# MarioAriasC/corda

Hardware: AMD Instinct MI355X
Metric: Ed25519 verifies/sec (node) (higher is better)
Workload: dtype uint32/uint64 (GF(2^255-19) radix 2^25.5 limbs, v_mad_u64_u32); 1 GPU; C2: 1M single-signer Ed25519 txs, 300-byte msg, distinct keys, SoA batch; sigs_per_gpu=1000000, msg_bytes=300, key_pool=distinct, parallelism=shard-by-signature x1, device_streams=2, gpu_max_hw_queues=4, collective=none

## Files before the change

### corda_amd/csrc/cv_field.h

```cpp
#pragma once
#include <hip/hip_runtime.h>
#include <stdint.h>
#include "cv_madc.h"

#define CV_HD __host__ __device__ __forceinline__

#if defined(CV_BOUNDS_CHECK) && !defined(__HIP_DEVICE_COMPILE__)
#include <cstdio>
#include <cstdlib>
#define CV_ASSERT(c, msg)                                                  \
    do {                                                                   \
        if (!(c)) {                                                        \
            fprintf(stderr, "cv_field bound violated: %s (%s:%d)\n", msg, __FILE__, __LINE__); \
            abort();                                                       \
        }                                                                  \
    } while (0)
#define CV_CHECKING 1
#else
#define CV_ASSERT(c, msg) ((void)0)
#define CV_CHECKING 0
#endif

struct fe { uint32_t v[10]; };

#define CV_W(i) (((i) & 1) ? 25 : 26)
#define CV_MASK(i) (((i) & 1) ? 0x1ffffffu : 0x3ffffffu)

#define CV_KP0(k) ((uint32_t)(k) * 0x3ffffedu)
#define CV_KPO(k) ((uint32_t)(k) * 0x1ffffffu)
#define CV_KPE(k) ((uint32_t)(k) * 0x3ffffffu)
CV_HD uint32_t cv_kp(int k, int i) { return i == 0 ? CV_KP0(k) : ((i & 1) ? CV_KPO(k) : CV_KPE(k)); }

CV_HD void fe_zero(fe &h) {
#pragma unroll
    for (int i = 0; i < 10; i++) h.v[i] = 0;
}
CV_HD void fe_one(fe &h) { fe_zero(h); h.v[0] = 1; }
CV_HD void fe_add(fe &h, const fe &f, const fe &g) {
#pragma unroll
    for (int i = 0; i < 10; i++) h.v[i] = f.v[i] + g.v[i];
}
template <int K> CV_HD void fe_sub(fe &h, const fe &f, const fe &g) {
#pragma unroll
    for (int i = 0; i < 10; i++) {
        CV_ASSERT(g.v[i] <= cv_kp(K, i), "fe_sub: subtrahend limb exceeds k*p");
        uint32_t k = cv_kp(K, i);
        const uint32_t x = g.v[i];
#ifdef __HIP_DEVICE_COMPILE__
        asm("" : "+s"(k));
#endif
        h.v[i] = (k > x ? k - x : x - k) + f.v[i];
    }
}
template <int K> CV_HD void fe_sub_carry_even(fe &h, const fe &f, const fe &g) {
#pragma unroll
    for (int i = 0; i < 10; i += 2) {
        uint32_t k0 = cv_kp(K, i), k1 = cv_kp(K, i + 1);
        CV_ASSERT(g.v[i] <= k0 && g.v[i + 1] <= k1, "fe_sub: subtrahend limb exceeds k*p");
#ifdef __HIP_DEVICE_COMPILE__
        asm("" : "+s"(k0), "+s"(k1));
#endif
        const uint32_t x0 = g.v[i], x1 = g.v[i + 1];
        const uint32_t e = (k0 > x0 ? k0 - x0 : x0 - k0) + f.v[i];
        uint32_t a1 = f.v[i + 1] + (e >> 26);
#ifdef __HIP_DEVICE_COMPILE__
        asm("" : "+v"(a1));
#endif
        h.v[i] = e & 0x3ffffffu;
        h.v[i + 1] = (k1 > x1 ? k1 - x1 : x1 - k1) + a1;
    }
}

CV_HD void fe_neg(fe &h, const fe &f) {
#pragma unroll
// ... 434 lines not shown
```

### corda_amd/csrc/cv_group.h

```cpp
#pragma once
#include "cv_field.h"

struct ge_p2 { fe X, Y, Z; };
struct ge_p3 { fe X, Y, Z, T; };
struct ge_p1p1 { fe X, Y, Z, T; };
struct ge_cached { fe YplusX, YminusX, Z, T2d; };
struct ge_precomp { fe yplusx, yminusx, xy2d; };

#define CV_FE_D   {56195235, 13857412, 51736253, 6949390, 114729, 24766616, 60832955, 30306712, 48412415, 21499315}
#define CV_FE_D2  {45281625, 27714825, 36363642, 13898781, 229458, 15978800, 54557047, 27058993, 29715967, 9444199}
#define CV_FE_SQRTM1 {34513072, 25610706, 9377949, 3500415, 12389472, 33281959, 41962654, 31548777, 326685, 11406482}

CV_HD void fe_const_d(fe &h) { const fe c = {CV_FE_D}; h = c; }
CV_HD void fe_const_d2(fe &h) { const fe c = {CV_FE_D2}; h = c; }
CV_HD void fe_const_sqrtm1(fe &h) { const fe c = {CV_FE_SQRTM1}; h = c; }

CV_HD void ge_p3_identity(ge_p3 &r) { fe_zero(r.X); fe_one(r.Y); fe_one(r.Z); fe_zero(r.T); }
CV_HD void ge_p2_identity(ge_p2 &r) { fe_zero(r.X); fe_one(r.Y); fe_one(r.Z); }
CV_HD void ge_cached_identity(ge_cached &r) { fe_one(r.YplusX); fe_one(r.YminusX); fe_one(r.Z); fe_zero(r.T2d); }
CV_HD void ge_precomp_identity(ge_precomp &r) { fe_one(r.yplusx); fe_one(r.yminusx); fe_zero(r.xy2d); }

CV_HD void ge_p1p1_to_p2(ge_p2 &r, const ge_p1p1 &p) {
    fe h[3];
    const fe f[3] = {p.T, p.Y, p.T}, g[3] = {p.X, p.Z, p.Z};
    fe_mul_n<3>(h, f, g);
    r.X = h[0]; r.Y = h[1]; r.Z = h[2];
}
CV_HD void ge_p1p1_to_p3(ge_p3 &r, const ge_p1p1 &p) {
    fe h[4];
    const fe f[4] = {p.T, p.Y, p.T, p.Y}, g[4] = {p.X, p.Z, p.Z, p.X};
    fe_mul_n<4>(h, f, g);
    r.X = h[0]; r.Y = h[1]; r.Z = h[2]; r.T = h[3];
}
CV_HD void ge_p3_to_p2(ge_p2 &r, const ge_p3 &p) { r.X = p.X; r.Y = p.Y; r.Z = p.Z; }
CV_HD void ge_p3_to_cached(ge_cached &r, const ge_p3 &p) {
    fe d2;
    fe_const_d2(d2);
    fe_add(r.YplusX, p.Y, p.X);
    fe_sub<2>(r.YminusX, p.Y, p.X);
    r.Z = p.Z;
    fe_mul(r.T2d, p.T, d2);
}

CV_HD void ge_p2_dbl(ge_p1p1 &r, const ge_p2 &p) {
    fe a, sq[4];
    fe_add(a, p.X, p.Y);
    const fe in[4] = {p.X, p.Y, p.Z, a};
    fe_sq_n<4, 0x4>(sq, in);
    const fe &xx = sq[0], &yy = sq[1], &zz2 = sq[2], &aa = sq[3];
    fe_add(r.Y, yy, xx);
    fe_sub<2>(r.Z, yy, xx);
    fe_sub_carry_even<3>(r.X, aa, r.Y);
    fe_sub<4>(r.T, zz2, r.Z);
}
CV_HD void ge_p3_dbl(ge_p1p1 &r, const ge_p3 &p) {
    ge_p2 q;
    ge_p3_to_p2(q, p);
    ge_p2_dbl(r, q);
}

CV_HD void ge_add(ge_p1p1 &r, const ge_p3 &p, const ge_cached &q) {
    fe s, d, m[4];
    fe_add(s, p.Y, p.X);
    fe_sub<2>(d, p.Y, p.X);
    const fe f[4] = {q.YplusX, q.YminusX, q.T2d, p.Z}, g[4] = {s, d, p.T, q.Z};
    fe_mul_n<4>(m, f, g);
    const fe &a = m[0], &b = m[1], &c = m[2];
    fe dd;
    fe_add(dd, m[3], m[3]);
    fe_sub<2>(r.X, a, b);
    fe_add(r.Y, a, b);
    fe_add(r.Z, dd, c);
    fe_sub<2>(r.T, dd, c);
}
CV_HD void ge_madd(ge_p1p1 &r, const ge_p3 &p, const ge_precomp &q) {
    fe s, d, m[3], dd;
    fe_add(s, p.Y, p.X);
    fe_sub<2>(d, p.Y, p.X);
    const fe f[3] = {q.yplusx, q.yminusx, q.xy2d}, g[3] = {s, d, p.T};
    fe_mul_n<3>(m, f, g);
    const fe &a = m[0], &b = m[1], &c = m[2];
    fe_add(dd, p.Z, p.Z);
    fe_sub<2>(r.X, a, b);
    fe_add(r.Y, a, b);
    fe_add(r.Z, dd, c);
    fe_sub<2>(r.T, dd, c);
}

CV_HD void ge_cached_cneg(ge_cached &r, bool neg) {
    fe a = r.YplusX, b = r.YminusX;
    fe_sel(r.YplusX, a, b, neg);
    fe_sel(r.YminusX, b, a, neg);
    uint32_t m = neg ? 0xffffffffu : 0u;
#ifdef __HIP_DEVICE_COMPILE__
    asm("" : "+v"(m));
#endif
#pragma unroll
    for (int i = 0; i < 10; i++) {
        CV_ASSERT(r.T2d.v[i] <= cv_kp(2, i), "ge_cached_cneg: 2dT limb exceeds 2p");
        r.T2d.v[i] = (r.T2d.v[i] ^ m) + (m & (cv_kp(2, i) + 1u));
    }
}
CV_HD void ge_precomp_cneg(ge_precomp &r, bool neg) {
    fe a = r.yplusx, b = r.yminusx, t;
    fe_sel(r.yplusx, a, b, neg);
    fe_sel(r.yminusx, b, a, neg);
    fe_neg(t, r.xy2d);
    fe_sel(r.xy2d, r.xy2d, t, neg);
}

__host__ __device__ __forceinline__ void ge_p2_encode(uint32_t w[8], const ge_p2 &p) {
    fe zi, x, y;
    fe_invert(zi, p.Z);
    fe_mul(x, p.X, zi);
    fe_mul(y, p.Y, zi);
    uint32_t xw[8];
    fe_to_words(w, y);
    fe_to_words(xw, x);
    w[7] |= (xw[0] & 1u) << 31;
}

CV_HD void ge_abyte_from_key(uint32_t abyte[8], const uint32_t w[8]) {
// ... 160 lines not shown
```

### corda_amd/csrc/cv_k_hs.hip

```cpp
#include "cv_kcommon.h"

template <int WAVES>
__global__ __launch_bounds__(CV_BLOCK, WAVES) void cv_scalars_kernel(uint32_t n, uint32_t cap, const uint8_t *__restrict__ pk,
                                                                 const uint8_t *__restrict__ sig,
                                                                 const uint8_t *__restrict__ arena,
                                                                 const uint64_t *__restrict__ off,
                                                                 const uint32_t *__restrict__ len,
                                                                 uint32_t *__restrict__ ws_dig) {
    const uint32_t i = blockIdx.x * CV_BLOCK + threadIdx.x;
    if (i < n) cv_scalars_lane<false, true>(i, cap, pk, sig, arena, off, len, ws_dig);
}

template <int WAVES, bool SUB>
__global__ __launch_bounds__(CV_BLOCK, WAVES) void cv_points_one_kernel(uint32_t n, const uint8_t *__restrict__ pk,
                                                                        const uint8_t *__restrict__ sig,
                                                                        uint32_t *__restrict__ ws_tab,
                                                                        uint32_t *__restrict__ ws_tabR,
                                                                        uint8_t *__restrict__ ws_ok,
                                                                        uint8_t *__restrict__ status) {
    cv_points_one_lane(blockIdx.x * CV_BLOCK + threadIdx.x, n, pk, sig, ws_tab, ws_tabR, ws_ok, status);
}

__global__ __launch_bounds__(CV_BLOCK) void cv_bw16_init_kernel(uint32_t *__restrict__ tab) {
    __shared__ __attribute__((aligned(16))) uint32_t btab[CV_BTAB_ENTRIES * CV_BTAB_STRIDE];
    stage_btab(btab);
    const uint32_t t = blockIdx.x * CV_BLOCK + threadIdx.x;
    if (t >= CV_BW16_ROWS * CV_BW16_ENTRIES) return;
    const uint32_t row = t / CV_BW16_ENTRIES, k = t % CV_BW16_ENTRIES;
    uint32_t sc[8] = {0, 0, 0, 0, 0, 0, 0, 0};
#pragma unroll
    for (int q = 0; q < 4; q++) sc[2 * q] = (uint32_t)q == row ? k : 0u;
    ge_p3 P;
    ge_scalarmult_base(P, sc, btab);
    fe zi, x, y, xy, d2, f[3];
    fe_invert(zi, P.Z);
    fe_mul(x, P.X, zi);
    fe_mul(y, P.Y, zi);
    fe_add(f[0], y, x);
    fe_sub<2>(f[1], y, x);
    fe_mul(xy, x, y);
    fe_const_d2(d2);
    fe_mul(f[2], xy, d2);
    uint32_t *o = tab + (size_t)t * CV_BTAB_STRIDE;
#pragma unroll
    for (int c = 0; c < 3; c++) {
        uint32_t w[8];
        fe_to_words(w, f[c]);
        fe canon;
        fe_from_words(canon, w);
        fe_store(o + 10 * c, canon);
    }
    o[30] = o[31] = 0;
}
template __global__ void cv_points_one_kernel<3, false>(uint32_t n, const uint8_t *pk, const uint8_t *sig, uint32_t *ws_tab, uint32_t *ws_tabR, uint8_t *ws_ok, uint8_t *status);
template __global__ void cv_points_one_kernel<3, true>(uint32_t n, const uint8_t *pk, const uint8_t *sig, uint32_t *ws_tab, uint32_t *ws_tabR, uint8_t *ws_ok, uint8_t *status);
template __global__ void cv_scalars_kernel<3>(uint32_t n, uint32_t cap, const uint8_t *pk, const uint8_t *sig, const uint8_t *arena, const uint64_t *off, const uint32_t *len, uint32_t *ws_dig);
```

### corda_amd/csrc/cv_kcommon.h

```cpp
#pragma once
#include <hip/hip_runtime.h>
#include <stdint.h>

#include "cv_verify.h"
#include "cv_quad.h"
#include "cv_hsquad.h"

#define CV_BLOCK 256
#ifndef CV_HSS_WAVES
#define CV_HSS_WAVES 3
#endif

__device__ __forceinline__ void stage_btab(uint32_t *lds) {
    for (int i = threadIdx.x; i < CV_BTAB_ENTRIES * CV_BTAB_STRIDE; i += blockDim.x) lds[i] = CV_BTAB[i];
    __syncthreads();
}

__device__ __forceinline__ void load_words8(uint32_t w[8], const uint8_t *p) {
    const uint4 a = reinterpret_cast<const uint4 *>(p)[0];
    const uint4 b = reinterpret_cast<const uint4 *>(p)[1];
    w[0] = a.x; w[1] = a.y; w[2] = a.z; w[3] = a.w;
    w[4] = b.x; w[5] = b.y; w[6] = b.z; w[7] = b.w;
}


__device__ __forceinline__ void store_words(uint32_t *dst, const uint32_t *src, int nwords4) {
    uint4 *d = reinterpret_cast<uint4 *>(dst);
#pragma unroll
    for (int q = 0; q < nwords4; q++) d[q] = make_uint4(src[4 * q], src[4 * q + 1], src[4 * q + 2], src[4 * q + 3]);
}

template <bool B16 = false, bool W16 = false>
__device__ __forceinline__ void cv_scalars_lane(uint32_t i, uint32_t cap, const uint8_t *pk, const uint8_t *sig,
                                                const uint8_t *arena, const uint64_t *off, const uint32_t *len,
                                                uint32_t *ws_dig) {
    uint32_t aw[8], rw[8], sw[8];
    load_words8(aw, pk + (size_t)i * 32);
    load_words8(rw, sig + (size_t)i * 64);
    load_words8(sw, sig + (size_t)i * 64 + 32);
    uint32_t hs[CV_HS_WORDS];
    cv_keyed_hs(aw, rw, sw, arena + off[i], len[i], hs);
    cv_hs_scalars<B16, W16>(hs, ws_dig + i, cap);
}

template <bool LAT = true>
__device__ __forceinline__ void cv_points_pair_lane(uint32_t g, uint32_t n, const uint8_t *pk, const uint8_t *sig,
                                                    uint32_t *ws_tab, uint32_t *ws_tabR, uint8_t *ws_ok,
                                                    uint8_t *status) {
    const uint32_t i = g >> 1;
    if (i >= n) return;
    const bool is_r = (g & 1u) != 0;
    uint32_t w[8];
    load_words8(w, is_r ? sig + (size_t)i * 64 : pk + (size_t)i * 32);
    const bool ok = cv_hs_point_one<LAT>(w, is_r, (is_r ? ws_tabR : ws_tab) + (size_t)i * CV_TAB_WORDS);
    const bool r_ok = __shfl_xor((int)ok, 1) != 0;
    if (!is_r) {
        ws_ok[i] = (ok && r_ok) ? 1 : 0;
        if (status) status[i] = ok ? 0 : 1;
    }
}

template <bool LAT = true>
__device__ __forceinline__ void cv_points_quad_lane(uint32_t g, uint32_t n, const uint8_t *pk, const uint8_t *sig,
                                                    uint32_t *ws_tab, uint32_t *ws_tabR, uint8_t *ws_ok,
                                                    uint8_t *status) {
    const uint32_t i = g >> 2;
    if (i >= n) return;
    const bool is_r = (g & 1u) != 0;
    const int half = (int)((g >> 1) & 1u);
    uint32_t w[8];
    load_words8(w, is_r ? sig + (size_t)i * 64 : pk + (size_t)i * 32);
    const bool ok = cv_hs_point_one<LAT>(w, is_r, (is_r ? ws_tabR : ws_tab) + (size_t)i * CV_TAB_WORDS, half);
    const bool r_ok = __shfl_xor((int)ok, 1) != 0;
    if (!is_r && half == 0) {
        ws_ok[i] = (ok && r_ok) ? 1 : 0;
        if (status) status[i] = ok ? 0 : 1;
    }
}

__device__ __forceinline__ void cv_points_one_lane(uint32_t g, uint32_t n, const uint8_t *pk, const uint8_t *sig,
                                                   uint32_t *ws_tab, uint32_t *ws_tabR, uint8_t *ws_ok,
                                                   uint8_t *status) {
    const uint32_t i = g >> 1;
    if (i >= n) return;
    const bool is_r = (g & 1u) != 0;
    uint32_t w[8];
    load_words8(w, is_r ? sig + (size_t)i * 64 : pk + (size_t)i * 32);
    const bool ok = cv_hs_point_one<false>(w, is_r, (is_r ? ws_tabR : ws_tab) + (size_t)i * CV_TAB_WORDS);
    const bool r_ok = __shfl_xor((int)ok, 1) != 0;
    if (!is_r) {
        ws_ok[i] = (ok && r_ok) ? 1 : 0;
        if (status) status[i] = ok ? 0 : 1;
    }
}
// ... 25 lines not shown
```

### corda_amd/csrc/cv_kernels.hip

```cpp
#include <hip/hip_runtime.h>
#include <stdint.h>

#include <mutex>

#include "cv_kcommon.h"
#include "cv_launch.h"

static uint32_t *g_bw16[64];
static std::mutex g_bw16_mu;
static hipError_t bw16_table(const uint32_t **out, hipStream_t st) {
    int dev = 0;
    hipError_t e = hipGetDevice(&dev);
    if (e != hipSuccess) return e;
    if (dev < 0 || dev >= 64) return hipErrorInvalidDevice;
    std::lock_guard<std::mutex> lk(g_bw16_mu);
    if (!g_bw16[dev]) {
        uint32_t *p = nullptr;
        if ((e = hipMalloc(&p, (size_t)CV_BW16_ROWS * CV_BW16_ROW * 4)) != hipSuccess) return e;
        hipLaunchKernelGGL(cv_bw16_init_kernel, dim3((CV_BW16_ROWS * CV_BW16_ENTRIES + CV_BLOCK - 1) / CV_BLOCK), dim3(CV_BLOCK),
                           0, st, p);
        if ((e = hipGetLastError()) == hipSuccess) e = hipStreamSynchronize(st);
        if (e != hipSuccess) {
            (void)hipFree(p);
            return e;
// ... 59 lines not shown
    if (ov) (void)hipStreamWaitEvent(po->aux, po->ready, 0);
    const uint32_t *bw16 = nullptr;
    if (n > plan->tri_max || n > plan->quad_max) {
        const hipError_t e = bw16_table(&bw16, stream);
        if (e != hipSuccess) return e;
    }
    uint32_t *ws_tabR = ws_tab + (size_t)ws_cap * CV_TAB_WORDS;
    for (uint32_t c0 = 0; c0 < n; c0 += ws_cap) {
        const uint32_t m = (n - c0 < ws_cap) ? n - c0 : ws_cap;
        const uint32_t blocks = (m + CV_BLOCK - 1) / CV_BLOCK;
        if (ev && c0 == 0) (void)hipEventRecord(ev[0], stream);
        if (n <= plan->quad_max) {
            const bool tri = m <= plan->tri_max;
            const uint32_t nbp = ((tri ? 4 : 2) * m + 63) / 64, nbs = (m + 63) / 64;
            if (ov) {
                if (tri) {
                    hipLaunchKernelGGL((cv_prep_lat_kernel<true, false>), dim3(nbp), dim3(64), 0, po->aux, m, ws_cap, nbp,
                                       1u, pk, sig, arena, off, len, ws_dig, ws_tab, ws_tabR, ws_ok, status, bitmap);
                    (void)hipEventRecord(po->done, po->aux);
                    hipLaunchKernelGGL((cv_prep_lat_kernel<true, false>), dim3(nbs), dim3(64), 0, stream, m, ws_cap, 0u, 1u,
                                       pk, sig, arena, off, len, ws_dig, ws_tab, ws_tabR, ws_ok, status, bitmap);
                } else {
                    hipLaunchKernelGGL((cv_prep_lat_kernel<false, false>), dim3(nbp), dim3(64), 0, po->aux, m, ws_cap, nbp,
                                       0u, pk, sig, arena, off, len, ws_dig, ws_tab, ws_tabR, ws_ok, status, bitmap);
                    (void)hipEventRecord(po->done, po->aux);
                    hipLaunchKernelGGL((cv_prep_lat_kernel<false, false>), dim3(nbs), dim3(64), 0, stream, m, ws_cap, 0u, 0u,
                                       pk, sig, arena, off, len, ws_dig, ws_tab, ws_tabR, ws_ok, status, bitmap);
                }
                (void)hipStreamWaitEvent(stream, po->done, 0);
            } else if (tri)
                hipLaunchKernelGGL((cv_prep_lat_kernel<true, false>), dim3(nbp + nbs), dim3(64), 0, stream, m, ws_cap, nbp, 1u,
                                   pk + (size_t)c0 * 32, sig + (size_t)c0 * 64, arena, off + c0, len + c0, ws_dig,
                                   ws_tab, ws_tabR, ws_ok, status ? status + c0 : nullptr, bitmap + (size_t)c0 / 64);
            else
                hipLaunchKernelGGL((cv_prep_lat_kernel<false, false>), dim3(nbp + nbs), dim3(64), 0, stream, m, ws_cap, nbp, 0u,
                                   pk + (size_t)c0 * 32, sig + (size_t)c0 * 64, arena, off + c0, len + c0, ws_dig,
                                   ws_tab, ws_tabR, ws_ok, status ? status + c0 : nullptr, bitmap + (size_t)c0 / 64);
            if (ev && c0 == 0) (void)hipEventRecord(ev[1], stream);
            if (ev && c0 == 0) (void)hipEventRecord(ev[2], stream);
            if (tri)
                hipLaunchKernelGGL(cv_hs_straus_tri_kernel<true>, dim3((16 * m + CV_BLOCK - 1) / CV_BLOCK), dim3(CV_BLOCK), 0,
                                   stream, m, ws_cap, ws_dig, ws_tab, ws_tabR, ws_ok, bitmap + (size_t)c0 / 64, nullptr);
            else if (!bw16)
                return hipErrorInvalidValue;
            else
                hipLaunchKernelGGL(cv_hs_straus_quad_kernel<true>, dim3((4 * m + CV_BLOCK - 1) / CV_BLOCK), dim3(CV_BLOCK),
                                   0, stream, m, ws_cap, ws_dig, ws_tab, ws_tabR, ws_ok, bitmap + (size_t)c0 / 64, bw16);
            if (ev && c0 == 0) (void)hipEventRecord(ev[3], stream);
            continue;
        }
        if (!bw16) return hipErrorInvalidValue;
        bool split = false;
        if (!ov && ax && ax->s2 && plan->split && !ev && m >= 131072) {
            const uint32_t resident = (uint32_t)ax->cus * 4u * 3u;
            const uint32_t last = ((m + 63) / 64) % resident;
            split = plan->split == 2 || (resident && last && last * 100u <= resident * 12u);
        }
        if (split) {
            const int pct = plan->split_pct >= 5 && plan->split_pct <= 50 ? plan->split_pct : 10;
            const uint32_t m1 = (uint32_t)(((uint64_t)m * (100 - pct) / 100) & ~(uint64_t)255);
            const uint32_t m2 = m - m1;
            const uint32_t sub0[2] = {0, m1}, subn[2] = {m1, m2};
            (void)hipEventRecord(ax->start, stream);
            (void)hipStreamWaitEvent(ax->s2, ax->start, 0);
            for (int h = 0; h < 2; h++) {
                hipStream_t st = h ? ax->s2 : stream;
                const uint32_t a = c0 + sub0[h], mm = subn[h], bl = (mm + CV_BLOCK - 1) / CV_BLOCK;
                launch_prep_tp<true>(mm, ws_cap, pk + (size_t)a * 32, sig + (size_t)a * 64, arena, off + a, len + a,
                                     ws_dig + sub0[h], ws_tab + (size_t)sub0[h] * CV_TAB_WORDS,
                                     ws_tabR + (size_t)sub0[h] * CV_TAB_WORDS, ws_ok + sub0[h],
                                     status ? status + a : nullptr, st, nullptr);
                hipLaunchKernelGGL((cv_hs_straus_kernel<CV_HSS_WAVES, true>), dim3(bl), dim3(CV_BLOCK), 0, st, mm, ws_cap,
                                   ws_dig + sub0[h], ws_tab + (size_t)sub0[h] * CV_TAB_WORDS,
                                   ws_tabR + (size_t)sub0[h] * CV_TAB_WORDS, ws_ok + sub0[h], bitmap + a / 64, bw16);
            }
            (void)hipEventRecord(ax->done2, ax->s2);
            (void)hipStreamWaitEvent(stream, ax->done2, 0);
            continue;
        }
        if (ov) {
            hipLaunchKernelGGL((cv_points_one_kernel<3, false>), dim3((2 * m + CV_BLOCK - 1) / CV_BLOCK), dim3(CV_BLOCK), 0,
                               po->aux, m, pk, sig, ws_tab, ws_tabR, ws_ok, status);
            (void)hipEventRecord(po->done, po->aux);
            hipLaunchKernelGGL(cv_scalars_kernel<3>, dim3(blocks), dim3(CV_BLOCK), 0, stream, m, ws_cap, pk, sig, arena, off,
                               len, ws_dig);
            (void)hipStreamWaitEvent(stream, po->done, 0);
            hipLaunchKernelGGL(cv_hs_straus_kernel<CV_HSS_WAVES>, dim3(blocks), dim3(CV_BLOCK), 0, stream, m, ws_cap, ws_dig, ws_tab,
                               ws_tabR, ws_ok, bitmap, bw16);
            continue;
        }
        launch_prep_tp<false>(m, ws_cap, pk + (size_t)c0 * 32, sig + (size_t)c0 * 64, arena, off + c0, len + c0, ws_dig,
                              ws_tab, ws_tabR, ws_ok, status ? status + c0 : nullptr, stream,
                              ev && c0 == 0 ? ev[1] : nullptr);
        if (ev && c0 == 0) (void)hipEventRecord(ev[2], stream);
        hipLaunchKernelGGL(cv_hs_straus_kernel<CV_HSS_WAVES>, dim3(blocks), dim3(CV_BLOCK), 0, stream, m, ws_cap, ws_dig, ws_tab,
                           ws_tabR, ws_ok, bitmap + (size_t)c0 / 64, bw16);
        if (ev && c0 == 0) (void)hipEventRecord(ev[3], stream);
    }
    return hipGetLastError();
}

hipError_t cvk_keyprep(uint32_t nk, const uint8_t *keys, const uint32_t *slots, uint32_t *scratch, uint32_t *ktab_pool,
                       uint8_t *kok_pool, hipStream_t stream) {
    if (nk == 0) return hipSuccess;
    hipLaunchKernelGGL(cv_keyprep_kernel, dim3((CV_COMB_ROWS * nk + CV_BLOCK - 1) / CV_BLOCK), dim3(CV_BLOCK), 0, stream, nk, keys,
                       slots, scratch, ktab_pool, kok_pool);
    return hipGetLastError();
// ... 102 lines not shown
```

### corda_amd/csrc/cv_sha.h

```cpp
#pragma once
#include "cv_field.h"

#define CV_K512_INIT { \
    0x428a2f98d728ae22ULL, 0x7137449123ef65cdULL, 0xb5c0fbcfec4d3b2fULL, 0xe9b5dba58189dbbcULL, \
    0x3956c25bf348b538ULL, 0x59f111f1b605d019ULL, 0x923f82a4af194f9bULL, 0xab1c5ed5da6d8118ULL, \
    0xd807aa98a3030242ULL, 0x12835b0145706fbeULL, 0x243185be4ee4b28cULL, 0x550c7dc3d5ffb4e2ULL, \
    0x72be5d74f27b896fULL, 0x80deb1fe3b1696b1ULL, 0x9bdc06a725c71235ULL, 0xc19bf174cf692694ULL, \
    0xe49b69c19ef14ad2ULL, 0xefbe4786384f25e3ULL, 0x0fc19dc68b8cd5b5ULL, 0x240ca1cc77ac9c65ULL, \
    0x2de92c6f592b0275ULL, 0x4a7484aa6ea6e483ULL, 0x5cb0a9dcbd41fbd4ULL, 0x76f988da831153b5ULL, \
    0x983e5152ee66dfabULL, 0xa831c66d2db43210ULL, 0xb00327c898fb213fULL, 0xbf597fc7beef0ee4ULL, \
    0xc6e00bf33da88fc2ULL, 0xd5a79147930aa725ULL, 0x06ca6351e003826fULL, 0x142929670a0e6e70ULL, \
    0x27b70a8546d22ffcULL, 0x2e1b21385c26c926ULL, 0x4d2c6dfc5ac42aedULL, 0x53380d139d95b3dfULL, \
    0x650a73548baf63deULL, 0x766a0abb3c77b2a8ULL, 0x81c2c92e47edaee6ULL, 0x92722c851482353bULL, \
    0xa2bfe8a14cf10364ULL, 0xa81a664bbc423001ULL, 0xc24b8b70d0f89791ULL, 0xc76c51a30654be30ULL, \
    0xd192e819d6ef5218ULL, 0xd69906245565a910ULL, 0xf40e35855771202aULL, 0x106aa07032bbd1b8ULL, \
    0x19a4c116b8d2d0c8ULL, 0x1e376c085141ab53ULL, 0x2748774cdf8eeb99ULL, 0x34b0bcb5e19b48a8ULL, \
    0x391c0cb3c5c95a63ULL, 0x4ed8aa4ae3418acbULL, 0x5b9cca4f7763e373ULL, 0x682e6ff3d6b2b8a3ULL, \
    0x748f82ee5defb2fcULL, 0x78a5636f43172f60ULL, 0x84c87814a1f0ab72ULL, 0x8cc702081a6439ecULL, \
    0x90befffa23631e28ULL, 0xa4506cebde82bde9ULL, 0xbef9a3f7b2c67915ULL, 0xc67178f2e372532bULL, \
    0xca273eceea26619cULL, 0xd186b8c721c0c207ULL, 0xeada7dd6cde0eb1eULL, 0xf57d4f7fee6ed178ULL, \
    0x06f067aa72176fbaULL, 0x0a637dc5a2c898a6ULL, 0x113f9804bef90daeULL, 0x1b710b35131c471bULL, \
    0x28db77f523047d84ULL, 0x32caab7b40c72493ULL, 0x3c9ebe0a15c9bebcULL, 0x431d67c49c100d4cULL, \
    0x4cc5d4becb3e42b6ULL, 0x597f299cfc657e2aULL, 0x5fcb6fab3ad6faecULL, 0x6c44198c4a475817ULL}
__device__ __constant__ static const uint64_t CV_K512_D[80] = CV_K512_INIT;
// ... 132 lines not shown
CV_HD void cv_msg_window(uint32_t dw[K], const uint8_t *msg, uint32_t mlen, uint32_t tstart) {
    const uint32_t sh = (uint32_t)((uintptr_t)msg & 3u);
    const uint32_t rem = mlen > tstart ? mlen - tstart + sh : 0u;
    const uint32_t kmax = rem >= 4u * K ? (uint32_t)K : (rem + 3) >> 2;
#pragma unroll
    for (int k = 0; k < K; k++) dw[k] = 0;
    if (kmax > 0) {
        const uint32_t *p = reinterpret_cast<const uint32_t *>(msg + tstart - sh);
#pragma unroll
        for (int k = 0; k < K; k++) {
            const uint32_t kk = (uint32_t)k < kmax ? (uint32_t)k : kmax - 1;
            dw[k] = p[kk];
        }
    }
}
CV_HD void sha512_msg_window(uint32_t dw[33], const uint8_t *msg, uint32_t mlen, uint32_t tstart) {
    cv_msg_window<33>(dw, msg, mlen, tstart);
}

template <int NPRE, bool FIRST>
CV_HD void sha512_block_words(uint64_t w[16], const uint32_t pre[16], const uint8_t *msg, uint32_t mlen, uint32_t blk,
                              uint32_t total, uint64_t bits) {
    const uint32_t tstart = FIRST ? 0u : blk * 128 - NPRE;
    uint32_t dw[33];
    sha512_msg_window(dw, msg, mlen, tstart);
    const uint32_t sh8 = 8u * (uint32_t)((uintptr_t)msg & 3u);
#pragma unroll
    for (int j = 0; j < 16; j++) {
        uint32_t d[2];
#pragma unroll
        for (int hl = 0; hl < 2; hl++) {
            const int jj = 2 * j + hl;
            const uint32_t u = blk * 128 + 4 * jj;
            uint32_t le;
            if (FIRST && jj < NPRE / 4) {
                le = pre[jj];
            } else {
                const int q = FIRST ? jj - NPRE / 4 : jj;
                const uint32_t t = u - NPRE;
                le = cv_funnel32(dw[q + 1], dw[q], sh8);
                const uint32_t valid = mlen - t;
                const uint32_t keep = valid >= 4 ? 0xffffffffu : ((1u << (8 * (valid & 3u))) - 1u);
                const uint32_t pad = valid >= 4 ? 0u : (0x80u << (8 * (valid & 3u)));
                le = (le & keep) | pad;
                if (t > mlen) le = 0;
            }
            d[hl] = cv_bswap32(le);
            if (u >= total - 8) d[hl] = (uint32_t)(bits >> (hl ? 0 : 32));
        }
        w[j] = ((uint64_t)d[0] << 32) | d[1];
    }
}

template <int NPRE>
__host__ __device__ __forceinline__ void sha512_pre_msg_t(uint32_t out[16], const uint32_t pre[16], const uint8_t *msg,
                                                          uint32_t mlen) {
    uint64_t st[8];
    sha512_init(st);
    const uint32_t data = NPRE + mlen;
    const uint32_t nblocks = (data + 1 + 16 + 127) / 128;
    const uint32_t total = nblocks * 128;
    const uint64_t bits = (uint64_t)data * 8;
    {
        uint64_t w[16];
        sha512_block_words<NPRE, true>(w, pre, msg, mlen, 0, total, bits);
        sha512_compress(st, w);
    }
#pragma nounroll
    for (uint32_t blk = 1; blk < nblocks; blk++) {
        uint64_t w[16];
        sha512_block_words<NPRE, false>(w, pre, msg, mlen, blk, total, bits);
        sha512_compress(st, w);
    }
#pragma unroll
    for (int i = 0; i < 8; i++) {
        out[2 * i] = cv_bswap32((uint32_t)(st[i] >> 32));
        out[2 * i + 1] = cv_bswap32((uint32_t)st[i]);
    }
}
__host__ __device__ __forceinline__ void sha512_pre_msg(uint32_t out[16], const uint32_t pre[16], int npre,
                                                        const uint8_t *msg, uint32_t mlen) {
    if (npre == 32) sha512_pre_msg_t<32>(out, pre, msg, mlen);
    else sha512_pre_msg_t<64>(out, pre, msg, mlen);
}

CV_HD void sha256_init(uint32_t st[8]) {
    st[0] = 0x6a09e667; st[1] = 0xbb67ae85; st[2] = 0x3c6ef372; st[3] = 0xa54ff53a;
    st[4] = 0x510e527f; st[5] = 0x9b05688c; st[6] = 0x1f83d9ab; st[7] = 0x5be0cd19;
}

__host__ __device__ __forceinline__ void sha256_compress(uint32_t st[8], uint32_t w[16]) {
    uint32_t a = st[0], b = st[1], c = st[2], d = st[3], e = st[4], f = st[5], g = st[6], h = st[7];
#pragma unroll
    for (int i = 0; i < 64; i++) {
        uint32_t wi;
        if (i < 16) {
            wi = w[i & 15];
        } else {
            const uint32_t x15 = w[(i - 15) & 15], x2 = w[(i - 2) & 15];
            const uint32_t s0 = cv_xor3(cv_ror32(x15, 7), cv_ror32(x15, 18), x15 >> 3);
            const uint32_t s1 = cv_xor3(cv_ror32(x2, 17), cv_ror32(x2, 19), x2 >> 10);
            wi = w[i & 15] + s0 + w[(i - 7) & 15] + s1;
            w[i & 15] = wi;
        }
        const uint32_t t1 = h + cv_xor3(cv_ror32(e, 6), cv_ror32(e, 11), cv_ror32(e, 25)) + ((e & f) ^ (~e & g)) +
                            cv_k256(i) + wi;
        const uint32_t t2 = cv_xor3(cv_ror32(a, 2), cv_ror32(a, 13), cv_ror32(a, 22)) + ((a & b) ^ (a & c) ^ (b & c));
        h = g; g = f; f = e; e = d + t1; d = c; c = b; b = a; a = t1 + t2;
    }
    st[0] += a; st[1] += b; st[2] += c; st[3] += d; st[4] += e; st[5] += f; st[6] += g; st[7] += h;
}

__host__ __device__ __forceinline__ void sha256_block_words(uint32_t w[16], const uint8_t *p, uint32_t n, uint32_t blk,
                                                            uint32_t total) {
    const uint64_t bits = (uint64_t)n * 8;
    const uint32_t sh8 = 8u * (uint32_t)((uintptr_t)p & 3u);
    uint32_t dw[17];
    cv_msg_window<17>(dw, p, n, blk * 64);
#pragma unroll
    for (int j = 0; j < 16; j++) {
        const uint32_t u = blk * 64 + 4 * j;
        uint32_t le = cv_funnel32(dw[j + 1], dw[j], sh8);
        const uint32_t valid = n - u;
        const uint32_t keep = valid >= 4 ? 0xffffffffu : ((1u << (8 * (valid & 3u))) - 1u);
// ... 40 lines not shown
```

### corda_amd/csrc/cv_verify.h

```cpp
#pragma once
#include "cv_field.h"
#include "cv_group.h"
#include "cv_scalar.h"
#include "cv_sha.h"
#include "cv_tables.h"

template <int STRIDE = CV_BTAB_STRIDE>
CV_HD void btab_select(ge_precomp &r, const uint32_t *btab, int k) {
    const int m = k < 0 ? -k : k;
    const uint4 *row = reinterpret_cast<const uint4 *>(btab + m * STRIDE);
    uint32_t t[32];
#pragma unroll
    for (int q = 0; q < 8; q++) {
        const uint4 v = row[q];
        t[4 * q] = v.x; t[4 * q + 1] = v.y; t[4 * q + 2] = v.z; t[4 * q + 3] = v.w;
    }
#pragma unroll
    for (int i = 0; i < 10; i++) {
        r.yplusx.v[i] = t[i];
        r.yminusx.v[i] = t[10 + i];
        r.xy2d.v[i] = t[20 + i];
    }
    ge_precomp_cneg(r, k < 0);
}
// ... 31 lines not shown
#define CV_TAB_WORDS (CV_TAB_ENTRIES * 40)
#define CV_HS_WORDS 16
#define CV_R_WORDS 32
#define CV_FIN_CHUNK 8
#define CV_BW16_ENTRIES 32769
#define CV_BW16_ROWS 4
#define CV_BW16_ROW (CV_BW16_ENTRIES * CV_BTAB_STRIDE)

CV_HD void fe_store(uint32_t *p, const fe &f) {
#pragma unroll
    for (int i = 0; i < 10; i++) p[i] = f.v[i];
}
CV_HD void fe_load(fe &f, const uint32_t *p) {
#pragma unroll
    for (int i = 0; i < 10; i++) f.v[i] = p[i];
}
CV_HD void ge_cached_store(uint32_t *p, const ge_cached &c) {
    fe_store(p, c.YplusX);
    fe_store(p + 10, c.YminusX);
    fe_store(p + 20, c.Z);
    fe_store(p + 30, c.T2d);
}
CV_HD void ge_cached_load(ge_cached &c, const uint32_t *p) {
    const uint4 *q = reinterpret_cast<const uint4 *>(p);
    uint32_t t[40];
#pragma unroll
    for (int j = 0; j < 10; j++) {
        const uint4 v = q[j];
        t[4 * j] = v.x; t[4 * j + 1] = v.y; t[4 * j + 2] = v.z; t[4 * j + 3] = v.w;
    }
    fe_load(c.YplusX, t);
    fe_load(c.YminusX, t + 10);
    fe_load(c.Z, t + 20);
    fe_load(c.T2d, t + 30);
}

CV_HD void ge_p3_neg(ge_p3 &r, const ge_p3 &a) {
    fe_neg(r.X, a.X);
    fe_carry(r.X, r.X);
    r.Y = a.Y;
    r.Z = a.Z;
    fe_neg(r.T, a.T);
    fe_carry(r.T, r.T);
}

__host__ __device__ __forceinline__ void ge_cached_multiples8(uint32_t *tab, const ge_p3 &P1) {
    ge_cached c1, c;
    ge_p3 P;
    ge_cached_identity(c);
    ge_cached_store(tab, c);
    ge_p3_to_cached(c1, P1);
    ge_cached_store(tab + 40, c1);
    ge_p1p1 t;
    ge_p3_dbl(t, P1);
    ge_p1p1_to_p3(P, t);
    ge_p3_to_cached(c, P);
    ge_cached_store(tab + 80, c);
#pragma unroll 1
    for (int k = 3; k <= 8; k++) {
        ge_add(t, P, c1);
        ge_p1p1_to_p3(P, t);
        ge_p3_to_cached(c, P);
        ge_cached_store(tab + 40 * k, c);
    }
}

__host__ __device__ __forceinline__ void ge_cached_multiples8_half(uint32_t *tab, const ge_p3 &P1, bool half1) {
    ge_cached c1, c2, c;
    ge_p3 Q;
    ge_p1p1 t;
    ge_p3_to_cached(c1, P1);
    ge_p3_dbl(t, P1);
    ge_p1p1_to_p3(Q, t);
    ge_p3_to_cached(c2, Q);
    if (half1) {
        ge_cached_store(tab + 80, c2);
    } else {
        ge_cached_identity(c);
        ge_cached_store(tab, c);
        ge_cached_store(tab + 40, c1);
    }
    ge_cached x;
    uint32_t m = half1 ? 0xffffffffu : 0u;
#ifdef __HIP_DEVICE_COMPILE__
    asm("" : "+v"(m));
#endif
#pragma unroll
    for (int i = 0; i < 10; i++) {
        x.YplusX.v[i] = (c2.YplusX.v[i] & m) | (c1.YplusX.v[i] & ~m);
        x.YminusX.v[i] = (c2.YminusX.v[i] & m) | (c1.YminusX.v[i] & ~m);
        x.Z.v[i] = (c2.Z.v[i] & m) | (c1.Z.v[i] & ~m);
        x.T2d.v[i] = (c2.T2d.v[i] & m) | (c1.T2d.v[i] & ~m);
    }
    const int k0 = half1 ? 4 : 3;
    ge_add(t, Q, x);
    ge_p1p1_to_p3(Q, t);
    ge_p3_to_cached(c, Q);
    ge_cached_store(tab + 40 * k0, c);
#pragma unroll
    for (int s = 1; s < 3; s++) {
        ge_add(t, Q, c2);
        ge_p1p1_to_p3(Q, t);
        ge_p3_to_cached(c, Q);
        ge_cached_store(tab + 40 * (k0 + 2 * s), c);
    }
}

template <bool LAT = false> __host__ __device__ __forceinline__ bool cv_verify_prep(const uint32_t aw[8], const uint32_t rw[8], const uint32_t sw[8],
                                               const uint8_t *msg, uint32_t mlen, uint32_t *hs, uint32_t *tab) {
    {
        uint32_t pre[16], dig[16], h[8], abyte[8];
        ge_abyte_from_key(abyte, aw);
#pragma unroll
        for (int q = 0; q < 8; q++) { pre[q] = rw[q]; pre[8 + q] = abyte[q]; }
        sha512_pre_msg(dig, pre, 64, msg, mlen);
        sc_reduce512(h, dig);
#pragma unroll
        for (int q = 0; q < 8; q++) hs[q] = h[q];
    }
    {
        uint32_t s[8];
        sc_effective_s(s, sw);
#pragma unroll
        for (int q = 0; q < 8; q++) hs[8 + q] = s[q];
    }
// ... 177 lines not shown
    for (int k = 2; k < CV_KENT_ENTRIES; k++) {
        fe_load(z, xrow + k * CV_KENT_WORDS + 20);
        fe_mul_m<true>(acc, acc, z);
        fe_store(trow + k * CV_KENT_WORDS + 20, acc);
    }
    fe inv, d2;
    fe_invert<true>(inv, acc);
    fe_const_d2(d2);
#pragma unroll 1
    for (int k = CV_KENT_ENTRIES - 1; k >= 1; k--) {
        fe zi, x, y, t;
        if (k > 1) {
            fe pre;
            fe_load(pre, trow + (k - 1) * CV_KENT_WORDS + 20);
            fe_mul_m<true>(zi, inv, pre);
            fe_load(z, xrow + k * CV_KENT_WORDS + 20);
            fe_mul_m<true>(inv, inv, z);
        } else {
            zi = inv;
        }
        fe_load(x, xrow + k * CV_KENT_WORDS);
        fe_load(y, xrow + k * CV_KENT_WORDS + 10);
        fe_mul_m<true>(x, x, zi);
        fe_mul_m<true>(y, y, zi);
        uint32_t *e = trow + k * CV_KENT_WORDS;
        fe_add(t, y, x);
        fe_carry(t, t);
        fe_store(e, t);
        fe_sub<2>(t, y, x);
        fe_carry(t, t);
        fe_store(e + 10, t);
        fe_mul_m<true>(t, x, y);
        fe_mul_m<true>(t, t, d2);
        fe_store(e + 20, t);
        e[30] = e[31] = 0;
    }
    {
        ge_precomp id;
        ge_precomp_identity(id);
        fe_store(trow, id.yplusx);
        fe_store(trow + 10, id.yminusx);
        fe_store(trow + 20, id.xy2d);
        trow[30] = trow[31] = 0;
    }
    return key_ok;
}

__host__ __device__ __forceinline__ bool cv_key_prep(const uint32_t aw[8], uint32_t *ext, uint32_t *ktab) {
    bool ok = true;
    for (int j = 0; j < CV_COMB_ROWS; j++) ok = cv_key_prep_row(aw, j, ext, ktab);
    return ok;
}

__host__ __device__ __forceinline__ void cv_keyed_hs(const uint32_t aw[8], const uint32_t rw[8], const uint32_t sw[8],
                                                     const uint8_t *msg, uint32_t mlen, uint32_t *hs) {
    uint32_t pre[16], dig[16], h[8], abyte[8], s[8];
    ge_abyte_from_key(abyte, aw);
#pragma unroll
    for (int q = 0; q < 8; q++) { pre[q] = rw[q]; pre[8 + q] = abyte[q]; }
    sha512_pre_msg(dig, pre, 64, msg, mlen);
    sc_reduce512(h, dig);
    sc_effective_s(s, sw);
#pragma unroll
    for (int q = 0; q < 8; q++) { hs[q] = h[q]; hs[8 + q] = s[q]; }
}

CV_HD void krow_select(ge_precomp &e, const uint32_t *row, int d) {
    const int m = d < 0 ? -d : d;
    const uint4 *q = reinterpret_cast<const uint4 *>(row + m * CV_KENT_WORDS);
    uint32_t t[32];
#pragma unroll
    for (int j = 0; j < 8; j++) {
        const uint4 v = q[j];
        t[4 * j] = v.x; t[4 * j + 1] = v.y; t[4 * j + 2] = v.z; t[4 * j + 3] = v.w;
    }
    fe_load(e.yplusx, t);
    fe_load(e.yminusx, t + 10);
    fe_load(e.xy2d, t + 20);
    ge_precomp_cneg(e, d < 0);
}

template <bool W16 = false>
__host__ __device__ __forceinline__ void cv_comb_straus(const uint32_t *bcomb, const uint32_t *hs, const uint32_t *ktab,
                                                        ge_p2 &out) {
    uint32_t h[8], s[8], sd[8];
#pragma unroll
    for (int q = 0; q < 8; q++) { h[q] = hs[q]; s[q] = hs[8 + q]; }
    if (W16) digits65536_pairs(sd, s);
    constexpr int NWIN = W16 ? 8 : 16, WBITS = W16 ? 8 : 4;
    ge_p2 R;
    ge_p2_identity(R);
#pragma unroll 1
    for (int u = NWIN - 1; u >= 0; u--) {
        ge_p1p1 t;
        ge_p3 R3;
        if (u != NWIN - 1) {
#pragma unroll 1
            for (int d = 0; d < WBITS - 1; d++) {
                ge_p2_dbl(t, R);
                ge_p1p1_to_p2(R, t);
            }
            ge_p2_dbl(t, R);
            ge_p1p1_to_p3(R3, t);
        } else {
            ge_p3_identity(R3);
        }
        const bool with_b = (u & 1) == 0;
#pragma unroll
        for (int j = 0; j < CV_COMB_ROWS; j++) {
            ge_precomp e;
            krow_select(e, ktab + j * CV_KROW_WORDS, W16 ? digit256_row(h, j, u) : digit16(h, 16 * j + u));
            ge_madd(t, R3, e);
            if (j + 1 < CV_COMB_ROWS || with_b) ge_p1p1_to_p3(R3, t);
// ... 486 lines not shown
```

Baseline: 110.4 million verifies/s.

## Add wave-uniform fast SHA-512 interior block loads and Z=1 doubling/add variants

Adds a fast path to SHA-512 message scheduling. When every lane in the wave has a full interior block, it loads aligned words and funnel-shifts them instead of running the generic byte-by-byte loader with padding logic. Adds Z=1 specialized point doubling and addition in the cached-multiples table builders, which skip a squaring and a multiply. The split heuristic now uses CV_HSS_WAVES instead of a hardcoded 3. The fast path reads up to 3 bytes past the message through an aligned-down pointer, and the Z=1 assumptions are only checked by debug asserts.

```diff
diff --git a/corda_amd/csrc/cv_field.h b/corda_amd/csrc/cv_field.h
--- a/corda_amd/csrc/cv_field.h
+++ b/corda_amd/csrc/cv_field.h
@@ -20,6 +20,14 @@
 #define CV_ASSERT(c, msg) ((void)0)
 #define CV_CHECKING 0
 #endif
+
+CV_HD bool cv_wave_all(bool p) {
+#ifdef __HIP_DEVICE_COMPILE__
+    return __all(p) != 0;
+#else
+    return p;
+#endif
+}
 
 struct fe { uint32_t v[10]; };
 
diff --git a/corda_amd/csrc/cv_group.h b/corda_amd/csrc/cv_group.h
--- a/corda_amd/csrc/cv_group.h
+++ b/corda_amd/csrc/cv_group.h
@@ -68,6 +68,43 @@
     const fe &a = m[0], &b = m[1], &c = m[2];
     fe dd;
     fe_add(dd, m[3], m[3]);
+    fe_sub<2>(r.X, a, b);
+    fe_add(r.Y, a, b);
+    fe_add(r.Z, dd, c);
+    fe_sub<2>(r.T, dd, c);
+}
+CV_HD bool fe_is_one_limbs(const fe &f) {
+    uint32_t o = f.v[0] ^ 1u;
+#pragma unroll
+    for (int i = 1; i < 10; i++) o |= f.v[i];
+    return o == 0;
+}
+
+CV_HD void ge_p3_dbl_z1(ge_p1p1 &r, const ge_p3 &p) {
+    CV_ASSERT(fe_is_one_limbs(p.Z), "ge_p3_dbl_z1: Z is not one");
+    fe a, sq[3], zz2;
+    fe_add(a, p.X, p.Y);
+    const fe in[3] = {p.X, p.Y, a};
+    fe_sq_n<3, 0>(sq, in);
+    const fe &xx = sq[0], &yy = sq[1], &aa = sq[2];
+    fe_zero(zz2);
+    zz2.v[0] = 2;
+    fe_add(r.Y, yy, xx);
+    fe_sub<2>(r.Z, yy, xx);
+    fe_sub_carry_even<3>(r.X, aa, r.Y);
+    fe_sub<4>(r.T, zz2, r.Z);
+}
+
+CV_HD void ge_add_z1(ge_p1p1 &r, const ge_p3 &p, const ge_cached &q) {
+    CV_ASSERT(fe_is_one_limbs(q.Z), "ge_add_z1: Z of the cached operand is not one");
+    fe s, d, m[3], z, dd;
+    fe_add(s, p.Y, p.X);
+    fe_sub<2>(d, p.Y, p.X);
+    const fe f[3] = {q.YplusX, q.YminusX, q.T2d}, g[3] = {s, d, p.T};
+    fe_mul_n<3>(m, f, g);
+    const fe &a = m[0], &b = m[1], &c = m[2];
+    fe_carry(z, p.Z);
+    fe_add(dd, z, z);
     fe_sub<2>(r.X, a, b);
     fe_add(r.Y, a, b);
     fe_add(r.Z, dd, c);
diff --git a/corda_amd/csrc/cv_k_hs.hip b/corda_amd/csrc/cv_k_hs.hip
--- a/corda_amd/csrc/cv_k_hs.hip
+++ b/corda_amd/csrc/cv_k_hs.hip
@@ -8,7 +8,7 @@
                                                                  const uint32_t *__restrict__ len,
                                                                  uint32_t *__restrict__ ws_dig) {
     const uint32_t i = blockIdx.x * CV_BLOCK + threadIdx.x;
-    if (i < n) cv_scalars_lane<false, true>(i, cap, pk, sig, arena, off, len, ws_dig);
+    if (i < n) cv_scalars_lane<false, true, true>(i, cap, pk, sig, arena, off, len, ws_dig);
 }
 
 template <int WAVES, bool SUB>
diff --git a/corda_amd/csrc/cv_kcommon.h b/corda_amd/csrc/cv_kcommon.h
--- a/corda_amd/csrc/cv_kcommon.h
+++ b/corda_amd/csrc/cv_kcommon.h
@@ -30,7 +30,7 @@
     for (int q = 0; q < nwords4; q++) d[q] = make_uint4(src[4 * q], src[4 * q + 1], src[4 * q + 2], src[4 * q + 3]);
 }
 
-template <bool B16 = false, bool W16 = false>
+template <bool B16 = false, bool W16 = false, bool FAST = false>
 __device__ __forceinline__ void cv_scalars_lane(uint32_t i, uint32_t cap, const uint8_t *pk, const uint8_t *sig,
                                                 const uint8_t *arena, const uint64_t *off, const uint32_t *len,
                                                 uint32_t *ws_dig) {
@@ -39,7 +39,7 @@
     load_words8(rw, sig + (size_t)i * 64);
     load_words8(sw, sig + (size_t)i * 64 + 32);
     uint32_t hs[CV_HS_WORDS];
-    cv_keyed_hs(aw, rw, sw, arena + off[i], len[i], hs);
+    cv_keyed_hs<FAST>(aw, rw, sw, arena + off[i], len[i], hs);
     cv_hs_scalars<B16, W16>(hs, ws_dig + i, cap);
 }
 
diff --git a/corda_amd/csrc/cv_kernels.hip b/corda_amd/csrc/cv_kernels.hip
--- a/corda_amd/csrc/cv_kernels.hip
+++ b/corda_amd/csrc/cv_kernels.hip
@@ -135,7 +135,7 @@
         if (!bw16) return hipErrorInvalidValue;
         bool split = false;
         if (!ov && ax && ax->s2 && plan->split && !ev && m >= 131072) {
-            const uint32_t resident = (uint32_t)ax->cus * 4u * 3u;
+            const uint32_t resident = (uint32_t)ax->cus * 4u * CV_HSS_WAVES;
             const uint32_t last = ((m + 63) / 64) % resident;
             split = plan->split == 2 || (resident && last && last * 100u <= resident * 12u);
         }
diff --git a/corda_amd/csrc/cv_sha.h b/corda_amd/csrc/cv_sha.h
--- a/corda_amd/csrc/cv_sha.h
+++ b/corda_amd/csrc/cv_sha.h
@@ -208,7 +208,45 @@
     }
 }
 
-template <int NPRE>
+template <int NPRE, bool FIRST>
+CV_HD bool sha512_block_interior(const uint8_t *msg, uint32_t mlen, uint32_t blk) {
+    constexpr uint32_t K = FIRST ? (128 - NPRE) / 4 + 1 : 33;
+    const uint32_t tstart = FIRST ? 0u : blk * 128 - NPRE;
+    const uint32_t sh = (uint32_t)((uintptr_t)msg & 3u);
+    return mlen >= tstart && mlen - tstart + (sh ? 1u : 0u) > 4u * (K - 1);
+}
+template <int NPRE, bool FIRST>
+CV_HD void sha512_block_words_interior(uint64_t w[16], const uint32_t pre[16], const uint8_t *msg, uint32_t blk) {
+    constexpr int Q0 = FIRST ? NPRE / 4 : 0;
+    constexpr int K = 32 - Q0 + 1;
+    const uint32_t tstart = FIRST ? 0u : blk * 128 - NPRE;
+    const uint32_t sh = (uint32_t)((uintptr_t)msg & 3u);
+    const uint32_t *p = reinterpret_cast<const uint32_t *>(msg + tstart - sh);
+    uint32_t dw[K];
+#pragma unroll
+    for (int k = 0; k < K; k++) dw[k] = p[k];
+    const uint32_t sh8 = 8u * sh;
+#pragma unroll
+    for (int j = 0; j < 16; j++) {
+        uint32_t d[2];
+#pragma unroll
+        for (int hl = 0; hl < 2; hl++) {
+            const int jj = 2 * j + hl;
+            d[hl] = cv_bswap32(jj < Q0 ? pre[jj] : cv_funnel32(dw[jj - Q0 + 1], dw[jj - Q0], sh8));
+        }
+        w[j] = ((uint64_t)d[0] << 32) | d[1];
+    }
+}
+template <int NPRE, bool FIRST, bool FAST>
+CV_HD void sha512_block_words_any(uint64_t w[16], const uint32_t pre[16], const uint8_t *msg, uint32_t mlen,
+                                  uint32_t blk, uint32_t total, uint64_t bits) {
+    if (FAST && cv_wave_all(sha512_block_interior<NPRE, FIRST>(msg, mlen, blk)))
+        sha512_block_words_interior<NPRE, FIRST>(w, pre, msg, blk);
+    else
+        sha512_block_words<NPRE, FIRST>(w, pre, msg, mlen, blk, total, bits);
+}
+
+template <int NPRE, bool FAST = false>
 __host__ __device__ __forceinline__ void sha512_pre_msg_t(uint32_t out[16], const uint32_t pre[16], const uint8_t *msg,
                                                           uint32_t mlen) {
     uint64_t st[8];
@@ -219,13 +257,13 @@
     const uint64_t bits = (uint64_t)data * 8;
     {
         uint64_t w[16];
-        sha512_block_words<NPRE, true>(w, pre, msg, mlen, 0, total, bits);
+        sha512_block_words_any<NPRE, true, FAST>(w, pre, msg, mlen, 0, total, bits);
         sha512_compress(st, w);
     }
 #pragma nounroll
     for (uint32_t blk = 1; blk < nblocks; blk++) {
         uint64_t w[16];
-        sha512_block_words<NPRE, false>(w, pre, msg, mlen, blk, total, bits);
+        sha512_block_words_any<NPRE, false, FAST>(w, pre, msg, mlen, blk, total, bits);
         sha512_compress(st, w);
     }
 #pragma unroll
diff --git a/corda_amd/csrc/cv_verify.h b/corda_amd/csrc/cv_verify.h
--- a/corda_amd/csrc/cv_verify.h
+++ b/corda_amd/csrc/cv_verify.h
@@ -107,13 +107,13 @@
     ge_p3_to_cached(c1, P1);
     ge_cached_store(tab + 40, c1);
     ge_p1p1 t;
-    ge_p3_dbl(t, P1);
+    ge_p3_dbl_z1(t, P1);
     ge_p1p1_to_p3(P, t);
     ge_p3_to_cached(c, P);
     ge_cached_store(tab + 80, c);
 #pragma unroll 1
     for (int k = 3; k <= 8; k++) {
-        ge_add(t, P, c1);
+        ge_add_z1(t, P, c1);
         ge_p1p1_to_p3(P, t);
         ge_p3_to_cached(c, P);
         ge_cached_store(tab + 40 * k, c);
@@ -125,7 +125,7 @@
     ge_p3 Q;
     ge_p1p1 t;
     ge_p3_to_cached(c1, P1);
-    ge_p3_dbl(t, P1);
+    ge_p3_dbl_z1(t, P1);
     ge_p1p1_to_p3(Q, t);
     ge_p3_to_cached(c2, Q);
     if (half1) {
@@ -409,13 +409,14 @@
     return ok;
 }
 
+template <bool FAST = false>
 __host__ __device__ __forceinline__ void cv_keyed_hs(const uint32_t aw[8], const uint32_t rw[8], const uint32_t sw[8],
                                                      const uint8_t *msg, uint32_t mlen, uint32_t *hs) {
     uint32_t pre[16], dig[16], h[8], abyte[8], s[8];
     ge_abyte_from_key(abyte, aw);
 #pragma unroll
     for (int q = 0; q < 8; q++) { pre[q] = rw[q]; pre[8 + q] = abyte[q]; }
-    sha512_pre_msg(dig, pre, 64, msg, mlen);
+    sha512_pre_msg_t<64, FAST>(dig, pre, msg, mlen);
     sc_reduce512(h, dig);
     sc_effective_s(s, sw);
 #pragma unroll
```

Result: no change. 111.2 million verifies/s, median of 6 (+0.7%).
